# yulong314/multi_camera_calibration

Measured on AMD Instinct MI355X. Metric: corner residual+Jacobian evals/sec + ms/LM-iter; RMS reproj-err vs ref, higher is better.
Workload: dtype f64; 1 GPU; config4: 4 omnidirectional cameras, 1000 synthetic 11x8-board views (BASELINE.json configs[3]), one Gauss-Newton step per 'step'; model=omnidirectional, cameras=4, views=1000, edges=3958, params=6018, parallelism=photo-sharded x1, transport=none, state_dtype=f32, jacobian_dtype=f64

## Files before the change

### multi_camera_calibration_amd/csrc/mcc_group.hpp

```cpp


template <int MODEL, bool BACK, int L, int GW = 28>
__device__ __forceinline__ void group_prologue(const double* ph, const double* ct, const double* sds, int side,
                                               int sub, double* S, double* P, double* Gb) {
    const double* R1 = ph;
    const double* Jr1 = ph + 9;
    const double* T1 = ph + 18;
    const double* R2 = ct;
    const double* Jl2 = ct + 9;
    const double* T2 = ct + 18;
    double* X = S;
    double* W = S + 15;
    for (int e = sub; e < 12; e += L) {
        if (e < 9) {
            const int i = e / 3, j = e % 3;
            X[e] = dot3_nc(R2[i * 3], R1[j], R2[i * 3 + 1], R1[3 + j], R2[i * 3 + 2], R1[6 + j]);
        } else {
            const int i = e - 9;
            const double q = dot3_nc(R2[i * 3], T1[0], R2[i * 3 + 1], T1[1], R2[i * 3 + 2], T1[2]);
            X[12 + i] = q;
            X[9 + i] = add_nc(q, T2[i]);
        }
    }
    wave_sync_lds();
// ... 569 lines not shown
                r[t - ntri] = v;
            }
        }
        if (tid < 2) norms[tid] = a.packed[ntri + 2 * m + tid];
        __syncthreads();
    }
    SSTAMP(srow, 3, 0);
    SolveCtx sc = a.solve;
    sc.stamps = srow;
    solve_global<false>(sc, S, r, norms[0], norms[1], nullptr, ivok ? Iv : nullptr, pre);
    SSTAMP(srow, 7, 0);
    fold_final_reset(la, src, have, useiv);
    SSTAMP_DRAINED(srow, 15, 0);
}
#ifndef MCC_FOLD_EARLY
#define MCC_FOLD_EARLY 1
#endif
template <int NT>
__device__ __forceinline__ void fold_final(const LinArgs& la) {
    __shared__ SolvePre s_pre;
    const SolvePre* pre = MCC_FOLD_EARLY ? &s_pre : nullptr;
    if (MCC_FOLD_EARLY && la.fsa.fuse_solve) {
        SolveCtx sc = la.fsa.solve;
        sc.stamps = la.fsa.stamps ? la.fsa.stamps + kSchurStampStride * (size_t)la.fold_parts : nullptr;
        solve_prefetch(sc, &s_pre);
    }
    if (NT == 512 && la.fold_direct) {
        fold_final_direct(la, pre);
        return;
    }
    constexpr int UM = kSchurOneLevelLoads * 256 / NT;
    const int n = 48 * la.fold_parts + (la.fsa.ssinv != nullptr ? la.fsa.m * la.fsa.m + 1 : 0);
    if (n <= UM / 2 * NT) fold_final_u<UM / 2>(la, pre);
    else fold_final_u<UM>(la, pre);
}

#ifndef MCC_GROUP_PAIR_THREADS
#define MCC_GROUP_PAIR_THREADS 256
#endif
#ifndef MCC_GROUP_OCC
#define MCC_GROUP_OCC 2
#endif
#ifndef MCC_EDGE_PRIO
#define MCC_EDGE_PRIO 2
#endif
template <int L, int AT>
__device__ __forceinline__ void edge_prio_up() {
    if (L == 32 && MCC_EDGE_PRIO == AT && __builtin_amdgcn_readfirstlane(threadIdx.x) >= 256) __builtin_amdgcn_s_setprio(1);
}
template <int L>
__device__ __forceinline__ void edge_prio_down() {
    if (L == 32 && MCC_EDGE_PRIO != 0) __builtin_amdgcn_s_setprio(0);
}
template <int MODEL, bool RATIONAL, int PRISM, bool BACK, int L>
__device__ __forceinline__ bool group_body(const LinArgs& a, const int grp) {
    constexpr int NT = kGroupRound * L, EPW = 64 / L;
    State* st = a.state;
    const int tid = threadIdx.x, lane = tid & 63, wave = tid >> 6;
    const int wv = __builtin_amdgcn_readfirstlane(wave);
    const int* __restrict__ hdr = a.ghdr + (size_t)kGHdrInts * grp;
    const int done = st->done, pending = st->pending;
    const double alpha_prev = st->alpha;
    const int p0 = hdr[kGHdrRange], np = hdr[kGHdrRange + 1];
    const int ge0 = hdr[kGHdrRange + 2], gne = hdr[kGHdrRange + 3];
    const int q0 = hdr[kGHdrRange + 4], nq = hdr[kGHdrRange + 5];
    const int c0 = hdr[kGHdrRange + 6], nc = hdr[kGHdrRange + 7];
    if (done) return false;
    long long* stp = a.stamps ? a.stamps + kStampStride * (size_t)grp : nullptr;
    SSTAMP(stp, 0, 0);
    const int C = a.n_cams, m = a.global_dim;
    extern __shared__ __attribute__((aligned(16))) double smem[];
    const GroupLayout GL = group_layout(gne, C, nq, nc);
#ifdef MCC_DIAG
    long long wt0 = 0, wt1 = 0, wt2 = 0, wt3 = 0;
#endif
    double* rec = smem + GL.rec;
    double* s27 = smem + GL.s27;
    double* sLi = smem + GL.sLi;
    double* sv = smem + GL.sv;
    double* sph = smem + GL.sph;
    double* sxn = smem + GL.sxn;
    double* spart = smem + GL.spart;
    double* sdg = smem + GL.sdg;
    double* ctab = smem + GL.ctab;
    double* ktab = smem + GL.ktab;
    double* sds = smem + GL.sds;
    double* sP = smem + GL.sP;
    double* sGb = smem + GL.sGb;
    int* ibase = reinterpret_cast<int*>(smem + GL.ndoubles);
    int4* sInfo = reinterpret_cast<int4*>(ibase + GL.iInfo);
    int* sgb = ibase + GL.iGb;
    int* seq = ibase + GL.iEq;
    int* sph0 = ibase + GL.iPh;
    int4* spq = reinterpret_cast<int4*>(ibase + GL.iPq);
    unsigned* scn = reinterpret_cast<unsigned*>(ibase + GL.iCn);
    float(*sC)[kGChunk][EPW] = reinterpret_cast<float(*)[kGChunk][EPW]>(smem + GL.sU + wave * (5 * kGChunk * EPW / 2));
    GroupChain* sCH = reinterpret_cast<GroupChain*>(smem + GL.sU + wave * (5 * kGChunk * EPW / 2));
    static_assert(EPW * sizeof(GroupChain) <= 5 * kGChunk * EPW * sizeof(float), "k_group chain union");

    const int g = lane % EPW, sub = lane / EPW;
    constexpr int PER = kGChunk / L;
    auto stage_load = [&](float (&v)[PER][5], int sb, int eoff, int cc0, int cn) {
#pragma unroll
        for (int u = 0; u < PER; ++u) {
            const int i = sb + L * u;
            const unsigned c = (unsigned)(eoff + cc0 + (i < cn ? i : 0));
            v[u][0] = a.obj_x[c];
            v[u][1] = a.obj_y[c];
            v[u][2] = a.obj_z[c];
            v[u][3] = a.img_u[c];
            v[u][4] = a.img_v[c];
        }
    };
    auto stage_store = [&](const float (&v)[PER][5], int sb, int cn) {
#pragma unroll
        for (int u = 0; u < PER; ++u) {
            const int i = sb + L * u;
            if (i < cn) {
#pragma unroll
                for (int f = 0; f < 5; ++f) sC[f][i][g] = v[u][f];
            }
        }
    };
    auto stage = [&](int eoff, int cc0, int cn) {
        float v[PER][5];
        int sb = sub;
        asm volatile("" : "+v"(sb));
        stage_load(v, sb, eoff, cc0, cn);
        stage_store(v, sb, cn);
    };

    constexpr int CAM0 = NT / 2, DST = CAM0 + 63;
    double om2[3] = {0.0, 0.0, 0.0}, T2[3] = {0.0, 0.0, 0.0};
    const int le0 = wave * EPW + g;
    const int4 info0 = *reinterpret_cast<const int4*>(hdr + kGHdrInfo + 4 * le0);
    int4 rInfo = make_int4(0, 0, 0, 0);
    int rGb = 0, rEq = 0, rPh = 0;
    if (wv == 0) {
        const int t = lane < kGroupRound ? lane : 0;
        rInfo = *reinterpret_cast<const int4*>(hdr + kGHdrInfo + 4 * t);
        rGb = hdr[kGHdrGb + t];
        rEq = hdr[kGHdrEq + t];
        rPh = hdr[kGHdrPhoto + (lane <= kPhotoGroup ? lane : 0)];
    }
    int4 rPq = make_int4(0, 0, 0, 0);
    unsigned rCn = 0;
    double rDg = 0.0, rKt = 0.0;
    if (wv * 64 < nq) rPq = a.gpairs[q0 + (tid < nq ? tid : 0)];
    if (wv * 64 < nc) rCn = a.gcon[c0 + (tid < nc ? tid : 0)];
    if (wv * 64 < m) rDg = a.dg[tid < m ? tid : 0];
    if (wv * 64 < kGIntr * C) rKt = a.kintr[tid < kGIntr * C ? tid : 0];
    float rCam[6] = {0.f, 0.f, 0.f, 0.f, 0.f, 0.f};
    double rDs[6] = {0.0, 0.0, 0.0, 0.0, 0.0, 0.0};
    if (wv == CAM0 / 64) {
        const int c = lane < C ? lane : 0;
        const float* src = MODEL == MCC_MODEL_DOUBLESIDE ? a.cam_rt + 6 * c : a.x + 6 * (c > 0 ? c - 1 : 0);
        if (BACK && MODEL == MCC_MODEL_DOUBLESIDE) src = tid == DST ? a.x : src;
#pragma unroll
        for (int k = 0; k < 6; ++k) rCam[k] = src[k];
        if (BACK && MODEL != MCC_MODEL_DOUBLESIDE) {
#pragma unroll
            for (int k = 0; k < 6; ++k) rDs[k] = a.ds_rt[k];
        }
    }
    float xo = 0.f;
    double zk = 0.0;
    const int pq = (tid - 192) / 6, pk = (tid - 192) % 6;
    const bool ptask = tid >= 192 && pq < np;
    double2 pn0 = make_double2(0.0, 0.0);
    if (wv == 3) {
        const size_t pi = ptask ? 6 * (size_t)(p0 + pq) + pk : 0;
        xo = a.x[m + pi];
        if (pending) zk = a.zp[pi];
        else if (a.fold) pn0 = *reinterpret_cast<const double2*>(a.photo_norm + (ptask && pk == 0 ? 2 * (size_t)(p0 + pq) : 0));
    }
    double y0[6] = {0.0, 0.0, 0.0, 0.0, 0.0, 0.0};
    int gb0 = -1;
    if (pending && wv * 64 < 6 * gne) {
        const bool act = tid < 6 * gne;
        const int le = act ? tid / 6 : 0, k = act ? tid % 6 : 0;
        gb0 = a.gblock[ge0 + le];
        const double* Ye = a.Y + 36 * (size_t)(ge0 + le);
#pragma unroll
        for (int i = 0; i < 6; ++i) y0[i] = Ye[6 * i + k];
    }
    float cv0[PER][5];
    int sb0 = sub;
    asm volatile("" : "+v"(sb0));
    const int cn0 = min(info0.w, kGChunk);
    __builtin_amdgcn_sched_barrier(0);
    stage_load(cv0, sb0, info0.z, 0, cn0);
    __builtin_amdgcn_sched_barrier(0);
#pragma unroll
    for (int k = 0; k < 6; ++k) asm volatile("" : "+v"(rCam[k]));
    if (wv == 0) {
        if (lane < kGroupRound && lane < gne) {
            sInfo[lane] = rInfo;
            sgb[lane] = rGb;
            seq[lane] = rEq;
        }
        if (lane <= np) sph0[lane] = rPh;
    }
    if (tid < nq) spq[tid] = rPq;
    if (tid < nc) scn[tid] = rCn;
    if (tid < m) sdg[tid] = rDg;
    if (tid < kGIntr * C) ktab[tid] = rKt;
    if (tid >= CAM0 && tid < CAM0 + C) {
        const bool fixed0 = MODEL != MCC_MODEL_DOUBLESIDE && tid == CAM0;
#pragma unroll
        for (int k = 0; k < 3; ++k) {
            om2[k] = fixed0 ? 0.0 : (double)rCam[k];
            T2[k] = fixed0 ? 0.0 : (double)rCam[3 + k];
        }
    } else if (BACK && tid == DST) {
#pragma unroll
        for (int k = 0; k < 3; ++k) {
            om2[k] = MODEL == MCC_MODEL_DOUBLESIDE ? (double)rCam[k] : rDs[k];
            T2[k] = MODEL == MCC_MODEL_DOUBLESIDE ? (double)rCam[3 + k] : rDs[3 + k];
        }
    }
#pragma unroll 1
    for (int t = kGroupRound + tid; t < gne; t += NT) {
        sInfo[t] = a.edge_info[ge0 + t];
        sgb[t] = a.gblock[ge0 + t];
        seq[t] = a.edge_lphoto[ge0 + t];
    }
#pragma unroll 1
    for (int t = NT + tid; t < nq; t += NT) spq[t] = a.gpairs[q0 + t];
#pragma unroll 1
    for (int t = NT + tid; t < nc; t += NT) scn[t] = a.gcon[c0 + t];
#pragma unroll 1
    for (int t = NT + tid; t < kGIntr * C; t += NT) ktab[t] = a.kintr[t];
    __syncthreads();
    SSTAMP(stp, 1, 0);
    if (pending) {
        for (int t = tid; t < 6 * gne; t += NT) {
            const int le = t / 6, k = t % 6;
            int gbl = gb0;
            double y[6];
            if (t == tid) {
#pragma unroll
                for (int i = 0; i < 6; ++i) y[i] = y0[i];
            } else {
                gbl = sgb[le];
                const double* Ye = a.Y + 36 * (size_t)(ge0 + le);
#pragma unroll
                for (int i = 0; i < 6; ++i) y[i] = Ye[6 * i + k];
            }
            const double* d = sdg + 6 * (gbl < 0 ? 0 : gbl);
            double sk = 0.0;
#pragma unroll
            for (int i = 0; i < 6; ++i) sk += y[i] * d[i];
            spart[6 * le + k] = gbl < 0 ? 0.0 : sk;
        }
    }
    __syncthreads();
    if (tid >= CAM0 && tid < CAM0 + C) {
        const int c = tid - CAM0;
        Rot r2;
        rodrigues_v2m(om2, r2);
        double J[9];
        so3_jac(om2, r2, +1.0, J);
        double* ct = ctab + 24 * c;
#pragma unroll
        for (int k = 0; k < 9; ++k) { ct[k] = r2.R[k]; ct[9 + k] = J[k]; }
#pragma unroll
        for (int k = 0; k < 3; ++k) ct[18 + k] = T2[k];
    } else if (BACK && tid == DST) {
        Rot rd;
        rodrigues_v2m(om2, rd);
        double J[9];
        so3_jac(om2, rd, -1.0, J);
#pragma unroll
        for (int k = 0; k < 9; ++k) { sds[k] = rd.R[k]; sds[9 + k] = J[k]; }
#pragma unroll
        for (int k = 0; k < 3; ++k) sds[18 + k] = T2[k];
    }
    if (ptask) {
        float xn = xo;
        double Gk = 0.0;
        if (pending) {
            double t = zk;
            for (int le = sph0[pq]; le < sph0[pq + 1]; ++le) t -= spart[6 * le + pk];
            const float G = (float)(alpha_prev * t);
            xn = xo + G;
            a.x[m + 6 * (size_t)(p0 + pq) + pk] = xn;
            Gk = (double)G;
        }
        sxn[16 * pq + pk] = (double)xn;
        sxn[16 * pq + 8 + pk] = Gk;
    }
    wave_sync_lds();
    if (ptask && pk == 0) {
        const double* xs = sxn + 16 * pq;
        if (pending) {
            double g2 = 0.0, x2 = 0.0;
#pragma unroll
            for (int q = 0; q < 6; ++q) {
                g2 += xs[8 + q] * xs[8 + q];
                x2 += xs[q] * xs[q];
            }
            a.photo_norm[2 * (size_t)(p0 + pq)] = g2;
            a.photo_norm[2 * (size_t)(p0 + pq) + 1] = x2;
            pn0 = make_double2(g2, x2);
        }
        if (a.fold) {
            sxn[16 * pq + 6] = pn0.x;
            sxn[16 * pq + 7] = pn0.y;
        }
        const double om1[3] = {xs[0], xs[1], xs[2]};
        Rot r1;
        rodrigues_v2m(om1, r1);
        double* ph = sph + 24 * pq;
        so3_jac(om1, r1, -1.0, ph + 9);
#pragma unroll
        for (int k = 0; k < 9; ++k) ph[k] = r1.R[k];
#pragma unroll
        for (int k = 0; k < 3; ++k) ph[18 + k] = xs[3 + k];
    }
    __syncthreads();
    SSTAMP(stp, 2, 0);
    WSTAMP(wt0);
    stage_store(cv0, sb0, cn0);

    for (int rb = 0; rb < gne; rb += kGroupRound) {
        const int es = wave * EPW + g, le = rb + es;
        const bool ev = le < gne;
        const int4 info = ev ? sInfo[le] : make_int4(0, 0, 0, 0);
        const int cam = info.x;
        double* P = sP + kGRecP * es;
        double* Gbe = sGb + 56 * es;
        edge_prio_up<L, 1>();
        if (rb > 0 && ev) stage(info.z, 0, min(info.w, kGChunk));
        if (ev) {
            group_prologue<MODEL, BACK, L>(sph + 24 * seq[le], ctab + 24 * cam, sds, info.y, sub, rec + kGRec * le, P, Gbe);
            const double* kt = ktab + kGIntr * cam;
            for (int k = sub; k < (PRISM == 2 ? 27 : 18); k += L) P[12 + k] = kt[k];
        }
        wave_sync_lds();
        if (rb == 0) SSTAMP(stp, 3, 0);
        if (rb == 0) WSTAMP(wt1);
        edge_prio_up<L, 2>();
        double acc[32];
#pragma unroll
        for (int q = 0; q < 32; ++q) acc[q] = 0.0;
        const int nn = info.w;
        for (int cc0 = 0;; cc0 += kGChunk) {
            if (cc0 >= nn) break;
            const int cn = min(nn - cc0, kGChunk);
            if (cc0 > 0) {
                wave_sync_lds();
                stage(info.z, cc0, cn);
                wave_sync_lds();
            }
#pragma unroll 1
            for (int i = sub; i < cn; i += L) {
                int po = 0;
                asm volatile("" : "+v"(po));
                const double* Pq = P + po;
                double R[9], T[3], kd[12];
#pragma unroll
                for (int q = 0; q < 9; ++q) R[q] = Pq[q];
#pragma unroll
                for (int q = 0; q < 3; ++q) T[q] = Pq[9 + q];
#pragma unroll
                for (int q = 0; q < 12; ++q) kd[q] = Pq[18 + q];
                const double fx = Pq[12], fy = Pq[13], cx = Pq[14], cy = Pq[15], sk = Pq[16], xi = Pq[17];
                const double X = sC[0][i][g], Y = sC[1][i][g], Z = sC[2][i][g];
                const float ou = sC[3][i][g], ov = sC[4][i][g];
                double Yr[3], D[6];
                float u, v;
                if (MODEL == MCC_MODEL_OMNI)
                    omni_corner(R, T, kd, fx, fy, cx, cy, sk, xi, X, Y, Z, Yr, u, v, D);
                else
                    pinhole_corner<RATIONAL, PRISM>(R, T, kd, fx, fy, cx, cy, X, Y, Z, Yr, u, v, D, Pq + 30);
                const float euf = ou - u, evf = ov - v;
                if (a.resid) {
                    const size_t c = (size_t)info.z + cc0 + i;
                    a.resid[2 * c] = euf;
                    a.resid[2 * c + 1] = evf;
                }
                const double eu = euf, ev2 = evf;
                double ju[6], jv[6];
                ju[0] = Yr[1] * D[2] - Yr[2] * D[1];
                ju[1] = Yr[2] * D[0] - Yr[0] * D[2];
                ju[2] = Yr[0] * D[1] - Yr[1] * D[0];
                ju[3] = D[0]; ju[4] = D[1]; ju[5] = D[2];
                jv[0] = Yr[1] * D[5] - Yr[2] * D[4];
                jv[1] = Yr[2] * D[3] - Yr[0] * D[5];
                jv[2] = Yr[0] * D[4] - Yr[1] * D[3];
                jv[3] = D[3]; jv[4] = D[4]; jv[5] = D[5];
                int q = 0;
#pragma unroll
                for (int r = 0; r < 6; ++r)
#pragma unroll
                    for (int s2 = r; s2 < 6; ++s2, ++q) acc[q] = fma(jv[r], jv[s2], fma(ju[r], ju[s2], acc[q]));
#pragma unroll
                for (int r = 0; r < 6; ++r) acc[21 + r] = fma(jv[r], ev2, fma(ju[r], eu, acc[21 + r]));
            }
        }
        if (rb == 0) SSTAMP(stp, 4, 0);
        if (rb == 0) WSTAMP(wt2);
        edge_prio_up<L, 3>();
        int tq = lane;
        asm volatile("" : "+v"(tq));
        strided_reduce_scatter<L>(acc, tq);
        const int gq = tq % EPW, sq = tq / EPW;
        const int base = strided_rs_base<L>(tq);
        wave_sync_lds();
        {
            GroupChain& CW = sCH[gq];
#pragma unroll
            for (int q = 0; q < 32 / L; ++q) {
                const int idx = base + q;
                if (idx < 21) {
                    int r, s2;
                    tri6(idx, r, s2);
                    CW.A[r * 6 + s2] = acc[q];
                    CW.A[s2 * 6 + r] = acc[q];
                } else if (idx < 27) {
                    CW.B[idx - 21] = acc[q];
                }
            }
        }
        wave_sync_lds();
        {
            const int eq = rb + wave * EPW + gq;
            group_chain(sCH[gq], sGb + 56 * (wave * EPW + gq), sq, eq < gne, rec + kGRec * (eq < gne ? eq : 0));
        }
        wave_sync_lds();
        edge_prio_down<L>();
        if (rb == 0) SSTAMP(stp, 5, 0);
        if (rb == 0) WSTAMP(wt3);
// ... 26 lines not shown
        const int q = tid, photo = p0 + q;
        double A[21], gs[6], Lm[6][6], Li[6][6];
        const double2* S2 = reinterpret_cast<const double2*>(s27 + 28 * q);
#pragma unroll
        for (int k = 0; k < 14; ++k) {
            const double2 w = S2[k];
            if (2 * k < 21) A[2 * k] = w.x; else gs[2 * k - 21] = w.x;
            if (2 * k + 1 < 21) A[2 * k + 1] = w.y; else if (2 * k + 1 < 27) gs[2 * k + 1 - 21] = w.y;
        }
        bool bad = false;
        double idg[6];
#pragma unroll
        for (int j = 0; j < 6; ++j) {
            double d = A[6 * j - j * (j - 1) / 2];
#pragma unroll
            for (int k = 0; k < j; ++k) d -= Lm[j][k] * Lm[j][k];
            bad |= !(d > 0.0);
            const double sd = sqrt(d > 0.0 ? d : 1.0);
            const double is = 1.0 / sd;
            Lm[j][j] = sd;
            idg[j] = is;
#pragma unroll
            for (int i = j + 1; i < 6; ++i) {
                double t = A[6 * j - j * (j - 1) / 2 + (i - j)];
#pragma unroll
                for (int k = 0; k < j; ++k) t -= Lm[i][k] * Lm[j][k];
                Lm[i][j] = t * is;
            }
        }
#pragma unroll
        for (int j = 0; j < 6; ++j) {
#pragma unroll
            for (int i = 0; i < 6; ++i) {
                if (i < j) { Li[i][j] = 0.0; continue; }
                double t = i == j ? 1.0 : 0.0;
#pragma unroll
                for (int k = j; k < i; ++k) t -= Lm[i][k] * Li[k][j];
                Li[i][j] = t * idg[i];
            }
        }
        double vv[6];
#pragma unroll
        for (int i = 0; i < 6; ++i) {
            double t = 0.0;
#pragma unroll
            for (int k = 0; k <= i; ++k) t += Li[i][k] * gs[k];
            vv[i] = t;
        }
#pragma unroll
        for (int j = 0; j < 6; ++j) {
            double t = 0.0;
#pragma unroll
            for (int i = j; i < 6; ++i) t += Li[i][j] * vv[i];
            a.zp[6 * (size_t)photo + j] = t;
            a.gp_tot[6 * (size_t)photo + j] = gs[j];
            sv[6 * q + j] = vv[j];
        }
        double2* L2 = reinterpret_cast<double2*>(sLi + 36 * q);
#pragma unroll
        for (int k = 0; k < 18; ++k) L2[k] = make_double2(Li[(2 * k) / 6][(2 * k) % 6], Li[(2 * k + 1) / 6][(2 * k + 1) % 6]);
        if (bad || photo == a.fault_photo) atomicOr(&st->error, kErrPhotoNotPD);
        if (a.fold) {
            double* fw = a.fnorm + 4 * (size_t)photo;
            st_sc1_x2(fw, sxn[16 * q + 6], sxn[16 * q + 7]);
            st_sc1(fw + 2, bad || photo == a.fault_photo ? 1.0 : 0.0);
        }
    }
    __syncthreads();
    SSTAMP(stp, 8, 0);
    for (int t = tid; t < 6 * gne; t += NT) {
        const int le = t / 6, i = t % 6;
        double h[6], li[36], u[6], y[6];
        double2* H2 = reinterpret_cast<double2*>(sE + ES * le + 22 + 6 * i);
        const double2* I2 = reinterpret_cast<const double2*>(sLi + 36 * seq[le]);
#pragma unroll
        for (int q = 0; q < 3; ++q) { const double2 w = H2[q]; h[2 * q] = w.x; h[2 * q + 1] = w.y; }
#pragma unroll
        for (int q = 0; q < 18; ++q) { const double2 w = I2[q]; li[2 * q] = w.x; li[2 * q + 1] = w.y; }
        const bool gl = sgb[le] >= 0;
#pragma unroll
        for (int j = 0; j < 6; ++j) {
            double w = 0.0;
#pragma unroll
            for (int k = 0; k <= j; ++k) w += h[k] * li[6 * j + k];
            u[j] = gl ? w : 0.0;
        }
#pragma unroll
        for (int j = 0; j < 6; ++j) {
            double w = 0.0;
#pragma unroll
            for (int k = j; k < 6; ++k) w += u[k] * li[6 * k + j];
            y[j] = w;
        }
        double2* G2 = reinterpret_cast<double2*>(a.Y + 36 * (size_t)(ge0 + le) + 6 * i);
#pragma unroll
        for (int q = 0; q < 3; ++q) {
            H2[q] = make_double2(u[2 * q], u[2 * q + 1]);
            G2[q] = make_double2(y[2 * q], y[2 * q + 1]);
        }
    }
    __syncthreads();
    SSTAMP(stp, 9, 0);
    int H = 1;
    while (H < 32 && 6 * nq * 2 * H <= (NT < MCC_GROUP_PAIR_THREADS ? NT : MCC_GROUP_PAIR_THREADS)) H *= 2;
    for (int t = tid; t < 6 * nq * H; t += NT) {
        const int h = t % H, k = t / H / 6, i0 = (t / H) % 6;
        const int4 pqv = spq[k];
        const bool diag = (pqv.z & 2) != 0;
        double acc[6], racc = 0.0, jacc = 0.0;
#pragma unroll
        for (int j = 0; j < 6; ++j) acc[j] = 0.0;
#pragma unroll 1
        for (int c = pqv.x + h; c < pqv.x + pqv.y; c += H) {
            const unsigned w = scn[c];
            const int ea = w & 255, eb = (w >> 8) & 255, q = w >> 17;
            const bool self = (w >> 16) & 1;
            const double2* Y2 = reinterpret_cast<const double2*>(sE + ES * ea + 22 + 6 * i0);
            const double2* B2 = reinterpret_cast<const double2*>(sE + ES * eb + 22);
            double y[6];
#pragma unroll
            for (int qq = 0; qq < 3; ++qq) { const double2 v = Y2[qq]; y[2 * qq] = v.x; y[2 * qq + 1] = v.y; }
            const double* Hgg = sE + ES * ea;
#pragma unroll
            for (int j = 0; j < 6; ++j) {
                double hb[6];
#pragma unroll
                for (int qq = 0; qq < 3; ++qq) { const double2 v = B2[3 * j + qq]; hb[2 * qq] = v.x; hb[2 * qq + 1] = v.y; }
                double d = 0.0;
#pragma unroll
                for (int kk = 0; kk < 6; ++kk) d += y[kk] * hb[kk];
                double hv = 0.0;
                if (self) {
                    const int rr = i0 < j ? i0 : j, cc = i0 < j ? j : i0;
                    hv = Hgg[rr * 6 - rr * (rr - 1) / 2 + (cc - rr)];
                }
                acc[j] += self ? hv - d : -d;
            }
            if (diag && self) {
                double d = 0.0;
#pragma unroll
                for (int kk = 0; kk < 6; ++kk) d += y[kk] * sv[6 * q + kk];
                const double gg = sE[ES * ea + 58 + i0];
                racc += gg - d;
                jacc += gg;
            }
        }
        for (int o = 1; o < H; o <<= 1) {
#pragma unroll
            for (int j = 0; j < 6; ++j) acc[j] += __shfl_xor(acc[j], o);
            racc += __shfl_xor(racc, o);
            jacc += __shfl_xor(jacc, o);
        }
        if (h == 0) {
            double* out = a.pairprod + (size_t)pqv.w;
#ifdef MCC_SLOT_PLAIN
#pragma unroll
            for (int j = 0; j < 6; ++j) out[i0 * 6 + j] = acc[j];
            if (diag) {
                out[36 + i0] = racc;
                out[42 + i0] = jacc;
            }
#else
#pragma unroll
            for (int j = 0; j < 6; j += 2) st_sc1_x2(out + i0 * 6 + j, acc[j], acc[j + 1]);
            if (diag) {
                st_sc1(out + 36 + i0, racc);
                st_sc1(out + 42 + i0, jacc);
            }
#endif
        }
    }
#ifdef MCC_DIAG
    asm volatile("s_waitcnt vmcnt(0)" ::: "memory");
    __syncthreads();
    SSTAMP(stp, 10, 0);
#endif
    return true;
}

template <int MODEL, bool RATIONAL, int PRISM, bool BACK, int L, bool FIRST = false>
__global__ __launch_bounds__(kGroupRound * L, MCC_GROUP_OCC * 16 / L) void k_group(LinArgs a) {
    constexpr int NT = kGroupRound * L;
    static_assert(L == 16 || L == 32, "k_group: 16 or 32 lanes per edge");
    State* st = a.state;
    const int tid = threadIdx.x;
    int grp = blockIdx.x;
    if (FIRST) {
        const int nlead = (int)gridDim.x - a.n_pgroups;
        grp = grp < nlead ? a.n_pgroups + grp : grp - nlead;
    }
    if (a.ssinv && grp == a.n_pgroups) {
        extern __shared__ __attribute__((aligned(16))) double smem_spare[];
        small_inverse(a, smem_spare, false);
        return;
    }
    int task;
    if (a.fold && grp > a.n_pgroups - (a.ssinv ? 0 : 1)) {
        if (st->done) return;
        task = grp - a.n_pgroups - (a.ssinv ? 1 : 0);
    } else {
        if (!group_body<MODEL, RATIONAL, PRISM, BACK, L>(a, grp) || PRISM == 2 || !a.fold_dyn) return;
        __shared__ int s_task;
        __syncthreads();
        if (tid == 0) {
            const int t = __hip_atomic_fetch_add(a.fold_ticket, 1, __ATOMIC_RELAXED, __HIP_MEMORY_SCOPE_AGENT);
            if (t == a.n_pgroups - 1) __hip_atomic_store(a.fold_ticket, 0, __ATOMIC_RELAXED, __HIP_MEMORY_SCOPE_AGENT);
            s_task = t;
        }
        __syncthreads();
        task = s_task;
    }
    if (task < a.fsa.n_items) fold_item(a, task);
    else if (task < a.fold_parts) fold_chunk(a, task - a.fsa.n_items);
    else if (task == a.fold_parts) fold_final<NT>(a);
}

#ifndef MCC_PREP4_WAVES
#define MCC_PREP4_WAVES 2
#endif
template <int MODEL, bool BACK>
__global__ __launch_bounds__(64, MCC_PREP4_WAVES) void k_prep4(LinArgs a) {
    const State* st = a.state;
    const int tid = threadIdx.x, grp = blockIdx.x;
    const int done = st->done, pending = st->pending;
    const double alpha_prev = st->alpha;
    const int p0 = a.prep_ptr[grp], np = a.prep_ptr[grp + 1] - p0;
    const int ge0 = a.prep_edge[grp], gne = a.prep_edge[grp + 1] - ge0;
    if (done) return;
    long long* stp = a.stamps ? a.stamps + kStampStride * (size_t)grp + 8 : nullptr;
    SSTAMP(stp, 0, 0);
    const int C = a.n_cams, m = a.global_dim;
    extern __shared__ __attribute__((aligned(16))) double smem[];
    const PrepLayout PL = prep_layout(C, BACK);
    double* tab = smem + PL.tab;
    double* S = smem + PL.S;
    double* spart = S;
    double* sdg = smem + PL.sdg;
    double* sxn = smem + PL.sxn;
    double* scam = smem + PL.scam;
    int* ib = reinterpret_cast<int*>(smem + PL.ndoubles);
    int4* sInfo = reinterpret_cast<int4*>(ib + PL.iInfo);
    int* sgb = ib + PL.iGb;
    int* sph0 = ib + PL.iPh;
    constexpr int SW = BACK ? 84 : 42;
    for (int t = tid; t < m; t += 64) sdg[t] = a.dg[t];
    for (int t = tid; t < 6 * C; t += 64) {
        const int c = t / 6, k = t % 6;
        scam[t] = MODEL == MCC_MODEL_DOUBLESIDE ? (double)a.cam_rt[t]
                                                : (c == 0 ? 0.0 : (double)a.x[6 * (c - 1) + k]);
    }
    if (BACK && tid < 6) scam[6 * C + tid] = MODEL == MCC_MODEL_DOUBLESIDE ? (double)a.x[tid] : a.ds_rt[tid];
    if (tid <= np) sph0[tid] = a.photo_ptr[p0 + tid] - ge0;
    for (int t = tid; t < gne; t += 64) {
        sInfo[t] = a.edge_info[ge0 + t];
        sgb[t] = a.gblock[ge0 + t];
    }
    const int pq = tid / 6, pk = tid % 6;
    const bool ptask = pq < np;
    float xo = 0.f;
    double zk = 0.0;
    double2 pn0 = make_double2(0.0, 0.0);
    if (ptask) {
        xo = a.x[m + 6 * (size_t)(p0 + pq) + pk];
        if (pending) zk = a.zp[6 * (size_t)(p0 + pq) + pk];
        else if (a.fold && pk == 0) pn0 = *reinterpret_cast<const double2*>(a.photo_norm + 2 * (size_t)(p0 + pq));
    }
    double y0[6];
// ... 100 lines not shown
```

### multi_camera_calibration_amd/csrc/mcc_internal.h

```cpp
#pragma once
#include <hip/hip_runtime.h>

#include "../../include/mcc.h"
#include "mcc_layout.hpp"

namespace mcc {

constexpr int kStampStride = 32;
constexpr int kSchurStampStride = 16;

struct State {
    int iter;
    int done;
    int crit_type;
    int max_count;
    double eps;
    double change;
    double alpha;
    double cam_normG2, cam_normX2;
    int error;
    int pending;
    unsigned int epoch;
    long long xchg_ticks;
    unsigned int spare_ack;
};
constexpr int kErrPhotoNotPD = 1;
constexpr int kErrCameraNotPD = 2;
constexpr int kErrPeerTimeout = 4;
constexpr int kErrWarmTimeout = 8;

struct PeerCtx {
    unsigned long long* inbox;
    unsigned long long* const* peers;
    int nranks;
    int rank, Lc;
    long long timeout;
};

struct SolveCtx {
    State* state;
    const double* alpha; int n_alpha;
    float* x;
    double* dg;
    double* delta;
    int m, do_update;
    long long* stamps;
    long long* sstats;
};

struct SchurArgs {
    State* state;
    const int4* items;
    const double* pairprod;
    double* item_out;
// ... 29 lines not shown
    const float* K; const float* D; const float* xi;
    const double* tilt;
    const float* cam_rt;
    const double* ds_rt;
    int nd, global_dim, n_cams, has_back;
    double* Y;
    const int* pgrp_ptr;
    const int* pgrp_edge;
    const unsigned char* edge_lphoto;
    const int* gpair_ptr;
    const int4* gpairs;
    const int* gcon_ptr;
    const unsigned* gcon;
    double* pairprod;
    int n_pgroups, max_gpairs, max_gcon, max_gedges;
    double* zp;
    double* gp_tot;
    float* resid;
    const int* gblock;
    const double* dg;
    double* photo_norm;
    long long* stamps;
    int fused, group_size, n_groups, rank, fuse_solve;
    double* contrib;
    double* gsum;
    int* cnt;
    double* packed;
    double* W;
    SolveCtx solve;
    PeerCtx peer;
    int n_edges, n_photos;
    double* erec;
    double* echain;
    double* eh;
    const int* prep_ptr;
    const int* prep_edge;
    int n_prep, prep_lanes;
    int fault_photo;
    int fold_first;
    double* ssinv;
    int* ssinv_ok;
    long long spare_wait, spare_delay;
    int fold, fold_parts;
    int fold_direct;
    int fold_dyn;
    int* fold_ticket;
    SchurArgs fsa;
    double* fnorm;
    double* fiv;
    const int* ghdr;
    const double* kintr;
};

struct WarmCtx {
    double* sinv;
    int* sinv_ok_sys;
    double* prev2;
    int prev_stride;
    int copy_prev;
    unsigned* sync;
    long long* stats;
    int poison;
    long long wait_ticks;
    long long idle_ticks;
    long long delay_ticks;
    int refine;
    double* xsol;
    int poll;
    long long* hst;
    int inv_la;
};
constexpr int kWarmMaxIters = 4;

struct SolveArgs {
    SolveCtx ctx;
    double* packed;
    PeerCtx peer;
    int pushed;
    WarmCtx warm;
};

struct BacksubArgs {
    const State* state;
    const int* photo_ptr;
    const int* gblock;
    const double* Y; const double* zp; const double* dg;
    const double* W;
    float* x;
    double* delta;
    double* photo_norm;
    int n_photos, m, do_update;
};

struct ErrArgs {
    const int4* edge_info;
    const int* edge_photo;
    const float* obj_x; const float* obj_y; const float* obj_z;
    const float* img_u; const float* img_v;
    const float* x;
    const float* K; const float* D; const float* xi;
    const double* tilt;
    const float* cam_pose;
    float* edge_sum;
    float* corner_err;
    int nd, m;
};
// ... 22 lines not shown
```

### multi_camera_calibration_amd/csrc/mcc_kernels.hip

```cpp
#include <array>
#include <map>
#include <mutex>
#include <hip/hip_runtime.h>

#include <algorithm>

#include "mcc_device.hpp"
#include "mcc_internal.h"

#ifdef MCC_PART
#define MCC_IN(n) (MCC_PART == (n))
#else
#define MCC_IN(n) 1
#endif
hipError_t mcc_attrs_linearize(size_t shmem);
hipError_t mcc_attrs_group16(size_t shmem);
hipError_t mcc_attrs_group32(size_t shmem);
hipError_t mcc_attrs_photo(size_t shmem);
hipError_t mcc_attrs_solve(size_t shmem);

namespace mcc {

#ifdef MCC_DIAG_RT
#define MCC_DIAG_CLOCK() __builtin_amdgcn_s_memrealtime()
// ... 4012 lines not shown
        if (p4) hipLaunchKernelGGL((k_prep4<MCC_MODEL_OMNI, false>), g4, dim3(64), p4shm, s, a);
        else hipLaunchKernelGGL((k_prep<MCC_MODEL_OMNI, false>), gp, dim3(64), 0, s, a);
        launch_edge<MCC_MODEL_OMNI, false, false>(a, s);
    } else if (model == MCC_MODEL_DOUBLESIDE) {
        if (p4) hipLaunchKernelGGL((k_prep4<MCC_MODEL_DOUBLESIDE, true>), g4, dim3(64), p4shm, s, a);
        else hipLaunchKernelGGL((k_prep<MCC_MODEL_DOUBLESIDE, true>), gp, dim3(64), 0, s, a);
        if (prism == 2) launch_edge<MCC_MODEL_DOUBLESIDE, true, 2>(a, s);
        else if (rational && prism) launch_edge<MCC_MODEL_DOUBLESIDE, true, true>(a, s);
        else if (rational) launch_edge<MCC_MODEL_DOUBLESIDE, true, false>(a, s);
        else if (prism) launch_edge<MCC_MODEL_DOUBLESIDE, false, true>(a, s);
        else launch_edge<MCC_MODEL_DOUBLESIDE, false, false>(a, s);
    } else {
        if (p4 && a.has_back) hipLaunchKernelGGL((k_prep4<MCC_MODEL_PINHOLE, true>), g4, dim3(64), p4shm, s, a);
        else if (p4) hipLaunchKernelGGL((k_prep4<MCC_MODEL_PINHOLE, false>), g4, dim3(64), p4shm, s, a);
        else if (a.has_back) hipLaunchKernelGGL((k_prep<MCC_MODEL_PINHOLE, true>), gp, dim3(64), 0, s, a);
        else hipLaunchKernelGGL((k_prep<MCC_MODEL_PINHOLE, false>), gp, dim3(64), 0, s, a);
        if (prism == 2) launch_edge<MCC_MODEL_PINHOLE, true, 2>(a, s);
        else if (rational && prism) launch_edge<MCC_MODEL_PINHOLE, true, true>(a, s);
        else if (rational) launch_edge<MCC_MODEL_PINHOLE, true, false>(a, s);
        else if (prism) launch_edge<MCC_MODEL_PINHOLE, false, true>(a, s);
        else launch_edge<MCC_MODEL_PINHOLE, false, false>(a, s);
    }
    hipLaunchKernelGGL(k_photo, dim3(a.n_pgroups), dim3(256), photo_shmem, s, a);
    return hipGetLastError();
}
hipError_t mcc_attrs_photo(size_t shmem) {
    return hipFuncSetAttribute((const void*)&k_photo, hipFuncAttributeMaxDynamicSharedMemorySize, (int)shmem);
}
#endif

#if MCC_IN(0)

size_t mcc_lin_shmem(int max_edges_per_photo, int n_cams, int m, int max_cpp) {
    const size_t lin = (size_t)max_edges_per_photo * sizeof(EdgeLds) + sizeof(PhotoLds) +
                       (kCamStride + kIntrStride) * sizeof(double) * (size_t)n_cams +
                       ((5 * sizeof(float) * (size_t)max_cpp + 15) & ~(size_t)15);
    return std::max(lin, (size_t)((m <= 30 ? 2 : 1) * m * m + m) * sizeof(double));
}

size_t mcc_solve_shmem(int m) {
    const size_t M = 16 * (size_t)((m + 15) / 16);
    const size_t blocked = M + M * (M + 1) + 2 * 16 * kBlkLd;
    const size_t warm = M <= kWarmN ? kWarmN + warm_shmem_doubles(m) : 0;
    const size_t helper = M <= kWarmN ? helper_shmem_doubles(m, true) : 0;
    return std::max((size_t)(m * m + m), m > 30 ? std::max(std::max(blocked, warm), helper) : 0) * sizeof(double);
}

#endif

#if MCC_IN(2) || MCC_IN(3)
template <int MODEL, bool RATIONAL, int PRISM, bool BACK, int L>
static hipError_t launch_group_t(const LinArgs& a, size_t shmem, hipStream_t s) {
    const dim3 grid(a.n_pgroups + (a.ssinv ? 1 : 0) + (a.fold && !a.fold_dyn ? a.fold_parts + 1 : 0));
    if (a.fold_first) {
        if (MODEL != MCC_MODEL_OMNI) return hipErrorInvalidValue;
        hipLaunchKernelGGL((k_group<MCC_MODEL_OMNI, false, false, false, L, true>), grid, dim3(kGroupRound * L), shmem, s, a);
        return hipGetLastError();
    }
    hipLaunchKernelGGL((k_group<MODEL, RATIONAL, PRISM, BACK, L>), grid, dim3(kGroupRound * L), shmem, s, a);
    return hipGetLastError();
}
template <int L>
static hipError_t launch_group_l(const LinArgs& a, int model, bool rational, int prism, size_t shmem, hipStream_t s) {
    if (model == MCC_MODEL_OMNI) return launch_group_t<MCC_MODEL_OMNI, false, false, false, L>(a, shmem, s);
    if (model == MCC_MODEL_DOUBLESIDE) {
        if (prism == 2) return launch_group_t<MCC_MODEL_DOUBLESIDE, true, 2, true, L>(a, shmem, s);
        if (rational && prism) return launch_group_t<MCC_MODEL_DOUBLESIDE, true, true, true, L>(a, shmem, s);
        if (rational) return launch_group_t<MCC_MODEL_DOUBLESIDE, true, false, true, L>(a, shmem, s);
        if (prism) return launch_group_t<MCC_MODEL_DOUBLESIDE, false, true, true, L>(a, shmem, s);
        return launch_group_t<MCC_MODEL_DOUBLESIDE, false, false, true, L>(a, shmem, s);
    }
    if (a.has_back) {
        if (prism == 2) return launch_group_t<MCC_MODEL_PINHOLE, true, 2, true, L>(a, shmem, s);
        if (rational && prism) return launch_group_t<MCC_MODEL_PINHOLE, true, true, true, L>(a, shmem, s);
        if (rational) return launch_group_t<MCC_MODEL_PINHOLE, true, false, true, L>(a, shmem, s);
        if (prism) return launch_group_t<MCC_MODEL_PINHOLE, false, true, true, L>(a, shmem, s);
        return launch_group_t<MCC_MODEL_PINHOLE, false, false, true, L>(a, shmem, s);
    }
    if (prism == 2) return launch_group_t<MCC_MODEL_PINHOLE, true, 2, false, L>(a, shmem, s);
    if (rational && prism) return launch_group_t<MCC_MODEL_PINHOLE, true, true, false, L>(a, shmem, s);
    if (rational) return launch_group_t<MCC_MODEL_PINHOLE, true, false, false, L>(a, shmem, s);
    if (prism) return launch_group_t<MCC_MODEL_PINHOLE, false, true, false, L>(a, shmem, s);
    return launch_group_t<MCC_MODEL_PINHOLE, false, false, false, L>(a, shmem, s);
}
template <int L>
static hipError_t set_group_attrs(size_t group_shmem) {
    hipError_t err = hipSuccess;
#define SETG(M, R, P, B) hipFuncSetAttribute((const void*)&k_group<M, R, P, B, L>, hipFuncAttributeMaxDynamicSharedMemorySize, (int)group_shmem)
    for (hipError_t e : {SETG(1, false, false, false), SETG(2, true, true, true), SETG(2, true, false, true),
                         SETG(2, false, true, true), SETG(2, false, false, true), SETG(0, true, true, true),
                         SETG(0, true, false, true), SETG(0, false, true, true), SETG(0, false, false, true),
                         SETG(0, true, true, false), SETG(0, true, false, false), SETG(0, false, true, false),
                         SETG(0, false, false, false), SETG(2, true, 2, true), SETG(0, true, 2, true),
                         SETG(0, true, 2, false),
                         hipFuncSetAttribute((const void*)&k_group<1, false, false, false, L, true>,
                                             hipFuncAttributeMaxDynamicSharedMemorySize, (int)group_shmem)})
        if (e != hipSuccess) err = e;
#undef SETG
    return err;
}
#endif
#if MCC_IN(3)
hipError_t mcc_launch_group32(const LinArgs& a, int model, bool rational, int prism, size_t shmem, hipStream_t s) {
    return launch_group_l<32>(a, model, rational, prism, shmem, s);
}
hipError_t mcc_attrs_group32(size_t shmem) { return set_group_attrs<32>(shmem); }
#endif
#if MCC_IN(2)
hipError_t mcc_launch_group32(const LinArgs& a, int model, bool rational, int prism, size_t shmem, hipStream_t s);
hipError_t mcc_launch_group(const LinArgs& a, int model, bool rational, int prism, int lanes, size_t shmem,
                            hipStream_t s) {
    if (a.n_photos <= 0 || a.n_edges <= 0) return hipSuccess;
// ... 119 lines not shown
```

Baseline: 14.31 billion corner evals/s.

## Restructure k_group kernel arguments into lead/hot blocks pinned in scalar registers

Splits k_group's single LinArgs argument into a 64-byte leading block of scalars, the full LinArgs, and a compact GroupHot struct of frequently used pointers. The kernel reads these straight from the kernarg segment at compile-time offsets and uses asm constraints to keep header values and pointers in SGPRs, with readfirstlane on the uniform state loads. The aim is to cut scalar load latency and vector register pressure in the group prologue. It also adds fragile offset bookkeeping guarded by static_asserts, and it enlarges the argument segment.

```diff
diff --git a/multi_camera_calibration_amd/csrc/mcc_group.hpp b/multi_camera_calibration_amd/csrc/mcc_group.hpp
--- a/multi_camera_calibration_amd/csrc/mcc_group.hpp
+++ b/multi_camera_calibration_amd/csrc/mcc_group.hpp
@@ -645,23 +645,60 @@
 __device__ __forceinline__ void edge_prio_down() {
     if (L == 32 && MCC_EDGE_PRIO != 0) __builtin_amdgcn_s_setprio(0);
 }
+template <class T>
+__device__ __forceinline__ T* pin_global(T* p) {
+    __attribute__((address_space(1))) T* g = (__attribute__((address_space(1))) T*)p;
+    asm volatile("" : "+s"(g));
+    return (T*)g;
+}
+__device__ __forceinline__ int first_lane(int v) { return __builtin_amdgcn_readfirstlane(v); }
+__device__ __forceinline__ double first_lane(double v) {
+    return __hiloint2double(first_lane(__double2hiint(v)), first_lane(__double2loint(v)));
+}
+template <class T>
+__device__ __forceinline__ const T& kernarg_at(const int off) {
+    typedef const __attribute__((address_space(4))) char* kbytes;
+    const __attribute__((address_space(4))) T* p =
+        (const __attribute__((address_space(4))) T*)((kbytes)__builtin_amdgcn_kernarg_segment_ptr() + off);
+    asm volatile("" : "+s"(p));
+    return *(const T*)p;
+}
 template <int MODEL, bool RATIONAL, int PRISM, bool BACK, int L>
-__device__ __forceinline__ bool group_body(const LinArgs& a, const int grp) {
+__device__ __forceinline__ bool group_body(State* st, const int* __restrict__ ghdr, const bool fold, const int grp,
+                                           const long long t_entry) {
     constexpr int NT = kGroupRound * L, EPW = 64 / L;
-    State* st = a.state;
     const int tid = threadIdx.x, lane = tid & 63, wave = tid >> 6;
     const int wv = __builtin_amdgcn_readfirstlane(wave);
-    const int* __restrict__ hdr = a.ghdr + (size_t)kGHdrInts * grp;
-    const int done = st->done, pending = st->pending;
-    const double alpha_prev = st->alpha;
-    const int p0 = hdr[kGHdrRange], np = hdr[kGHdrRange + 1];
-    const int ge0 = hdr[kGHdrRange + 2], gne = hdr[kGHdrRange + 3];
-    const int q0 = hdr[kGHdrRange + 4], nq = hdr[kGHdrRange + 5];
-    const int c0 = hdr[kGHdrRange + 6], nc = hdr[kGHdrRange + 7];
+    const int* __restrict__ hdr = ghdr + (size_t)kGHdrInts * grp;
+    int done = first_lane(st->done), pending = first_lane(st->pending);
+    double alpha_prev = first_lane(st->alpha);
+    int p0 = first_lane(hdr[kGHdrRange]), np = first_lane(hdr[kGHdrRange + 1]);
+    int ge0 = first_lane(hdr[kGHdrRange + 2]), gne = first_lane(hdr[kGHdrRange + 3]);
+    int q0 = first_lane(hdr[kGHdrRange + 4]), nq = first_lane(hdr[kGHdrRange + 5]);
+    int c0 = first_lane(hdr[kGHdrRange + 6]), nc = first_lane(hdr[kGHdrRange + 7]);
+    GroupHot hp = kernarg_at<GroupHot>(kGArgHot);
+    asm volatile("" ::"s"(done), "s"(pending), "s"(alpha_prev), "s"(p0), "s"(np), "s"(ge0), "s"(gne), "s"(q0), "s"(nq),
+                 "s"(c0), "s"(nc), "s"(hp.gpairs), "s"(hp.gcon), "s"(hp.dg), "s"(hp.kintr), "s"(hp.x), "s"(hp.cam_rt),
+                 "s"(hp.ds_rt), "s"(hp.zp), "s"(hp.photo_norm), "s"(hp.gblock), "s"(hp.Y), "s"(hp.obj_x), "s"(hp.obj_y),
+                 "s"(hp.obj_z), "s"(hp.img_u), "s"(hp.img_v), "s"(hp.stamps), "s"(hp.global_dim), "s"(hp.n_cams));
+    asm volatile("" ::"s"(hp.edge_info), "s"(hp.edge_lphoto), "s"(hp.gp_tot), "s"(hp.resid));
+    asm volatile("" : "+s"(done), "+s"(pending), "+s"(alpha_prev), "+s"(p0), "+s"(np), "+s"(ge0), "+s"(gne), "+s"(q0),
+                 "+s"(nq), "+s"(c0), "+s"(nc), "+s"(hp.global_dim), "+s"(hp.n_cams));
+    hp.gpairs = pin_global(hp.gpairs); hp.gcon = pin_global(hp.gcon); hp.dg = pin_global(hp.dg);
+    hp.kintr = pin_global(hp.kintr); hp.x = pin_global(hp.x); hp.cam_rt = pin_global(hp.cam_rt);
+    hp.ds_rt = pin_global(hp.ds_rt); hp.zp = pin_global(hp.zp); hp.photo_norm = pin_global(hp.photo_norm);
+    hp.gblock = pin_global(hp.gblock); hp.Y = pin_global(hp.Y); hp.obj_x = pin_global(hp.obj_x);
+    hp.obj_y = pin_global(hp.obj_y); hp.obj_z = pin_global(hp.obj_z); hp.img_u = pin_global(hp.img_u);
+    hp.img_v = pin_global(hp.img_v); hp.stamps = pin_global(hp.stamps);
+    hp.edge_info = pin_global(hp.edge_info); hp.edge_lphoto = pin_global(hp.edge_lphoto);
+    hp.gp_tot = pin_global(hp.gp_tot); hp.resid = pin_global(hp.resid);
     if (done) return false;
-    long long* stp = a.stamps ? a.stamps + kStampStride * (size_t)grp : nullptr;
+    long long* stp = hp.stamps ? hp.stamps + kStampStride * (size_t)grp : nullptr;
     SSTAMP(stp, 0, 0);
-    const int C = a.n_cams, m = a.global_dim;
+#ifdef MCC_DIAG
+    if (stp && (tid == 0 || tid == NT - 64)) stp[tid == 0 ? 12 : 13] = t_entry;
+#endif
+    const int C = hp.n_cams, m = hp.global_dim;
     extern __shared__ __attribute__((aligned(16))) double smem[];
     const GroupLayout GL = group_layout(gne, C, nq, nc);
 #ifdef MCC_DIAG
@@ -698,11 +735,11 @@
         for (int u = 0; u < PER; ++u) {
             const int i = sb + L * u;
             const unsigned c = (unsigned)(eoff + cc0 + (i < cn ? i : 0));
-            v[u][0] = a.obj_x[c];
-            v[u][1] = a.obj_y[c];
-            v[u][2] = a.obj_z[c];
-            v[u][3] = a.img_u[c];
-            v[u][4] = a.img_v[c];
+            v[u][0] = hp.obj_x[c];
+            v[u][1] = hp.obj_y[c];
+            v[u][2] = hp.obj_z[c];
+            v[u][3] = hp.img_u[c];
+            v[u][4] = hp.img_v[c];
         }
     };
     auto stage_store = [&](const float (&v)[PER][5], int sb, int cn) {
@@ -739,21 +776,21 @@
     int4 rPq = make_int4(0, 0, 0, 0);
     unsigned rCn = 0;
     double rDg = 0.0, rKt = 0.0;
-    if (wv * 64 < nq) rPq = a.gpairs[q0 + (tid < nq ? tid : 0)];
-    if (wv * 64 < nc) rCn = a.gcon[c0 + (tid < nc ? tid : 0)];
-    if (wv * 64 < m) rDg = a.dg[tid < m ? tid : 0];
-    if (wv * 64 < kGIntr * C) rKt = a.kintr[tid < kGIntr * C ? tid : 0];
+    if (wv * 64 < nq) rPq = hp.gpairs[q0 + (tid < nq ? tid : 0)];
+    if (wv * 64 < nc) rCn = hp.gcon[c0 + (tid < nc ? tid : 0)];
+    if (wv * 64 < m) rDg = hp.dg[tid < m ? tid : 0];
+    if (wv * 64 < kGIntr * C) rKt = hp.kintr[tid < kGIntr * C ? tid : 0];
     float rCam[6] = {0.f, 0.f, 0.f, 0.f, 0.f, 0.f};
     double rDs[6] = {0.0, 0.0, 0.0, 0.0, 0.0, 0.0};
     if (wv == CAM0 / 64) {
         const int c = lane < C ? lane : 0;
-        const float* src = MODEL == MCC_MODEL_DOUBLESIDE ? a.cam_rt + 6 * c : a.x + 6 * (c > 0 ? c - 1 : 0);
-        if (BACK && MODEL == MCC_MODEL_DOUBLESIDE) src = tid == DST ? a.x : src;
+        const float* src = MODEL == MCC_MODEL_DOUBLESIDE ? hp.cam_rt + 6 * c : hp.x + 6 * (c > 0 ? c - 1 : 0);
+        if (BACK && MODEL == MCC_MODEL_DOUBLESIDE) src = tid == DST ? hp.x : src;
 #pragma unroll
         for (int k = 0; k < 6; ++k) rCam[k] = src[k];
         if (BACK && MODEL != MCC_MODEL_DOUBLESIDE) {
 #pragma unroll
-            for (int k = 0; k < 6; ++k) rDs[k] = a.ds_rt[k];
+            for (int k = 0; k < 6; ++k) rDs[k] = hp.ds_rt[k];
         }
     }
     float xo = 0.f;
@@ -763,17 +800,17 @@
     double2 pn0 = make_double2(0.0, 0.0);
     if (wv == 3) {
         const size_t pi = ptask ? 6 * (size_t)(p0 + pq) + pk : 0;
-        xo = a.x[m + pi];
-        if (pending) zk = a.zp[pi];
-        else if (a.fold) pn0 = *reinterpret_cast<const double2*>(a.photo_norm + (ptask && pk == 0 ? 2 * (size_t)(p0 + pq) : 0));
+        xo = hp.x[m + pi];
+        if (pending) zk = hp.zp[pi];
+        else if (fold) pn0 = *reinterpret_cast<const double2*>(hp.photo_norm + (ptask && pk == 0 ? 2 * (size_t)(p0 + pq) : 0));
     }
     double y0[6] = {0.0, 0.0, 0.0, 0.0, 0.0, 0.0};
     int gb0 = -1;
     if (pending && wv * 64 < 6 * gne) {
         const bool act = tid < 6 * gne;
         const int le = act ? tid / 6 : 0, k = act ? tid % 6 : 0;
-        gb0 = a.gblock[ge0 + le];
-        const double* Ye = a.Y + 36 * (size_t)(ge0 + le);
+        gb0 = hp.gblock[ge0 + le];
+        const double* Ye = hp.Y + 36 * (size_t)(ge0 + le);
 #pragma unroll
         for (int i = 0; i < 6; ++i) y0[i] = Ye[6 * i + k];
     }
@@ -814,18 +851,19 @@
     }
 #pragma unroll 1
     for (int t = kGroupRound + tid; t < gne; t += NT) {
-        sInfo[t] = a.edge_info[ge0 + t];
-        sgb[t] = a.gblock[ge0 + t];
-        seq[t] = a.edge_lphoto[ge0 + t];
+        sInfo[t] = hp.edge_info[ge0 + t];
+        sgb[t] = hp.gblock[ge0 + t];
+        seq[t] = hp.edge_lphoto[ge0 + t];
     }
 #pragma unroll 1
-    for (int t = NT + tid; t < nq; t += NT) spq[t] = a.gpairs[q0 + t];
+    for (int t = NT + tid; t < nq; t += NT) spq[t] = hp.gpairs[q0 + t];
 #pragma unroll 1
-    for (int t = NT + tid; t < nc; t += NT) scn[t] = a.gcon[c0 + t];
+    for (int t = NT + tid; t < nc; t += NT) scn[t] = hp.gcon[c0 + t];
 #pragma unroll 1
-    for (int t = NT + tid; t < kGIntr * C; t += NT) ktab[t] = a.kintr[t];
+    for (int t = NT + tid; t < kGIntr * C; t += NT) ktab[t] = hp.kintr[t];
     __syncthreads();
     SSTAMP(stp, 1, 0);
+    const LinArgs& a = kernarg_at<LinArgs>(kGArgLin);
     if (pending) {
         for (int t = tid; t < 6 * gne; t += NT) {
             const int le = t / 6, k = t % 6;
@@ -836,7 +874,7 @@
                 for (int i = 0; i < 6; ++i) y[i] = y0[i];
             } else {
                 gbl = sgb[le];
-                const double* Ye = a.Y + 36 * (size_t)(ge0 + le);
+                const double* Ye = hp.Y + 36 * (size_t)(ge0 + le);
 #pragma unroll
                 for (int i = 0; i < 6; ++i) y[i] = Ye[6 * i + k];
             }
@@ -877,7 +915,7 @@
             for (int le = sph0[pq]; le < sph0[pq + 1]; ++le) t -= spart[6 * le + pk];
             const float G = (float)(alpha_prev * t);
             xn = xo + G;
-            a.x[m + 6 * (size_t)(p0 + pq) + pk] = xn;
+            hp.x[m + 6 * (size_t)(p0 + pq) + pk] = xn;
             Gk = (double)G;
         }
         sxn[16 * pq + pk] = (double)xn;
@@ -893,11 +931,11 @@
                 g2 += xs[8 + q] * xs[8 + q];
                 x2 += xs[q] * xs[q];
             }
-            a.photo_norm[2 * (size_t)(p0 + pq)] = g2;
-            a.photo_norm[2 * (size_t)(p0 + pq) + 1] = x2;
+            hp.photo_norm[2 * (size_t)(p0 + pq)] = g2;
+            hp.photo_norm[2 * (size_t)(p0 + pq) + 1] = x2;
             pn0 = make_double2(g2, x2);
         }
-        if (a.fold) {
+        if (fold) {
             sxn[16 * pq + 6] = pn0.x;
             sxn[16 * pq + 7] = pn0.y;
         }
@@ -968,10 +1006,10 @@
                 else
                     pinhole_corner<RATIONAL, PRISM>(R, T, kd, fx, fy, cx, cy, X, Y, Z, Yr, u, v, D, Pq + 30);
                 const float euf = ou - u, evf = ov - v;
-                if (a.resid) {
+                if (hp.resid) {
                     const size_t c = (size_t)info.z + cc0 + i;
-                    a.resid[2 * c] = euf;
-                    a.resid[2 * c + 1] = evf;
+                    hp.resid[2 * c] = euf;
+                    hp.resid[2 * c + 1] = evf;
                 }
                 const double eu = euf, ev2 = evf;
                 double ju[6], jv[6];
@@ -1104,15 +1142,15 @@
             double t = 0.0;
 #pragma unroll
             for (int i = j; i < 6; ++i) t += Li[i][j] * vv[i];
-            a.zp[6 * (size_t)photo + j] = t;
-            a.gp_tot[6 * (size_t)photo + j] = gs[j];
+            hp.zp[6 * (size_t)photo + j] = t;
+            hp.gp_tot[6 * (size_t)photo + j] = gs[j];
             sv[6 * q + j] = vv[j];
         }
         double2* L2 = reinterpret_cast<double2*>(sLi + 36 * q);
 #pragma unroll
         for (int k = 0; k < 18; ++k) L2[k] = make_double2(Li[(2 * k) / 6][(2 * k) % 6], Li[(2 * k + 1) / 6][(2 * k + 1) % 6]);
         if (bad || photo == a.fault_photo) atomicOr(&st->error, kErrPhotoNotPD);
-        if (a.fold) {
+        if (fold) {
             double* fw = a.fnorm + 4 * (size_t)photo;
             st_sc1_x2(fw, sxn[16 * q + 6], sxn[16 * q + 7]);
             st_sc1(fw + 2, bad || photo == a.fault_photo ? 1.0 : 0.0);
@@ -1144,7 +1182,7 @@
             for (int k = j; k < 6; ++k) w += u[k] * li[6 * k + j];
             y[j] = w;
         }
-        double2* G2 = reinterpret_cast<double2*>(a.Y + 36 * (size_t)(ge0 + le) + 6 * i);
+        double2* G2 = reinterpret_cast<double2*>(hp.Y + 36 * (size_t)(ge0 + le) + 6 * i);
 #pragma unroll
         for (int q = 0; q < 3; ++q) {
             H2[q] = make_double2(u[2 * q], u[2 * q + 1]);
@@ -1231,40 +1269,50 @@
 }
 
 template <int MODEL, bool RATIONAL, int PRISM, bool BACK, int L, bool FIRST = false>
-__global__ __launch_bounds__(kGroupRound * L, MCC_GROUP_OCC * 16 / L) void k_group(LinArgs a) {
+__global__ __launch_bounds__(kGroupRound * L, MCC_GROUP_OCC * 16 / L) void k_group(
+    State* st, const int* ghdr, const int n_pgroups, const unsigned flags, const int n_items, const int fold_parts,
+    long long, long long, long long, long long, LinArgs, GroupHot) {
     constexpr int NT = kGroupRound * L;
     static_assert(L == 16 || L == 32, "k_group: 16 or 32 lanes per edge");
-    State* st = a.state;
+    static_assert(GSame<decltype(&k_group<MODEL, RATIONAL, PRISM, BACK, L, FIRST>), GroupKernelFn>::v,
+                  "k_group's parameters are GroupKernelFn's: kernarg_at's offsets are computed from that list");
+    long long t_entry = 0;
+    WSTAMP(t_entry);
     const int tid = threadIdx.x;
+    const bool spare = (flags & kGLeadSsinv) != 0, fold = (flags & kGLeadFold) != 0;
     int grp = blockIdx.x;
     if (FIRST) {
-        const int nlead = (int)gridDim.x - a.n_pgroups;
-        grp = grp < nlead ? a.n_pgroups + grp : grp - nlead;
-    }
-    if (a.ssinv && grp == a.n_pgroups) {
+        const int nlead = (int)gridDim.x - n_pgroups;
+        grp = grp < nlead ? n_pgroups + grp : grp - nlead;
+    }
+    if (spare && grp == n_pgroups) {
         extern __shared__ __attribute__((aligned(16))) double smem_spare[];
-        small_inverse(a, smem_spare, false);
+        small_inverse(kernarg_at<LinArgs>(kGArgLin), smem_spare, false);
         return;
     }
     int task;
-    if (a.fold && grp > a.n_pgroups - (a.ssinv ? 0 : 1)) {
+    if (fold && grp > n_pgroups - (spare ? 0 : 1)) {
         if (st->done) return;
-        task = grp - a.n_pgroups - (a.ssinv ? 1 : 0);
+        task = grp - n_pgroups - (spare ? 1 : 0);
     } else {
-        if (!group_body<MODEL, RATIONAL, PRISM, BACK, L>(a, grp) || PRISM == 2 || !a.fold_dyn) return;
+        if (!group_body<MODEL, RATIONAL, PRISM, BACK, L>(st, ghdr, fold, grp, t_entry) || PRISM == 2 ||
+            !(flags & kGLeadFoldDyn))
+            return;
         __shared__ int s_task;
         __syncthreads();
         if (tid == 0) {
-            const int t = __hip_atomic_fetch_add(a.fold_ticket, 1, __ATOMIC_RELAXED, __HIP_MEMORY_SCOPE_AGENT);
-            if (t == a.n_pgroups - 1) __hip_atomic_store(a.fold_ticket, 0, __ATOMIC_RELAXED, __HIP_MEMORY_SCOPE_AGENT);
+            int* ticket = kernarg_at<LinArgs>(kGArgLin).fold_ticket;
+            const int t = __hip_atomic_fetch_add(ticket, 1, __ATOMIC_RELAXED, __HIP_MEMORY_SCOPE_AGENT);
+            if (t == n_pgroups - 1) __hip_atomic_store(ticket, 0, __ATOMIC_RELAXED, __HIP_MEMORY_SCOPE_AGENT);
             s_task = t;
         }
         __syncthreads();
         task = s_task;
     }
-    if (task < a.fsa.n_items) fold_item(a, task);
-    else if (task < a.fold_parts) fold_chunk(a, task - a.fsa.n_items);
-    else if (task == a.fold_parts) fold_final<NT>(a);
+    const LinArgs& a = kernarg_at<LinArgs>(kGArgLin);
+    if (task < n_items) fold_item(a, task);
+    else if (task < fold_parts) fold_chunk(a, task - n_items);
+    else if (task == fold_parts) fold_final<NT>(a);
 }
 
 #ifndef MCC_PREP4_WAVES
diff --git a/multi_camera_calibration_amd/csrc/mcc_internal.h b/multi_camera_calibration_amd/csrc/mcc_internal.h
--- a/multi_camera_calibration_amd/csrc/mcc_internal.h
+++ b/multi_camera_calibration_amd/csrc/mcc_internal.h
@@ -1,5 +1,7 @@
 #pragma once
 #include <hip/hip_runtime.h>
+
+#include <cstddef>
 
 #include "../../include/mcc.h"
 #include "mcc_layout.hpp"
@@ -135,6 +137,82 @@
     const double* kintr;
 };
 
+constexpr unsigned kGLeadSsinv = 1u, kGLeadFold = 2u, kGLeadFoldDyn = 4u, kGLeadFoldDirect = 8u;
+constexpr int kGLeadPreload = 6;
+struct GroupLead {
+    State* state;
+    const int* ghdr;
+    int n_pgroups;
+    unsigned flags;
+    int n_items;
+    int fold_parts;
+    long long pad[4];
+};
+static_assert(sizeof(GroupLead) == 64 && sizeof(GroupLead) % alignof(LinArgs) == 0,
+              "k_group: LinArgs follows the leading block at byte 64 of the argument segment");
+inline GroupLead group_lead(const LinArgs& a) {
+    return {a.state, a.ghdr, a.n_pgroups,
+            (a.ssinv ? kGLeadSsinv : 0u) | (a.fold ? kGLeadFold : 0u) | (a.fold_dyn ? kGLeadFoldDyn : 0u) |
+                (a.fold_direct ? kGLeadFoldDirect : 0u),
+            a.fsa.n_items, a.fold_parts, {0, 0, 0, 0}};
+}
+struct GroupHot {
+    const int4* gpairs;
+    const unsigned* gcon;
+    const double* dg;
+    const double* kintr;
+    float* x;
+    const float* cam_rt;
+    const double* ds_rt;
+    double* zp;
+    double* photo_norm;
+    const int* gblock;
+    double* Y;
+    const float* obj_x; const float* obj_y; const float* obj_z;
+    const float* img_u; const float* img_v;
+    long long* stamps;
+    const int4* edge_info;
+    const unsigned char* edge_lphoto;
+    double* gp_tot;
+    float* resid;
+    int global_dim, n_cams;
+};
+inline GroupHot group_hot(const LinArgs& a) {
+    return {a.gpairs, a.gcon, a.dg, a.kintr, a.x, a.cam_rt, a.ds_rt, a.zp, a.photo_norm, a.gblock, a.Y,
+            a.obj_x, a.obj_y, a.obj_z, a.img_u, a.img_v, a.stamps, a.edge_info, a.edge_lphoto, a.gp_tot, a.resid,
+            a.global_dim, a.n_cams};
+}
+using GroupKernelFn = void (*)(State*, const int*, int, unsigned, int, int, long long, long long, long long, long long,
+                               LinArgs, GroupHot);
+template <class T, class U> struct GSame { static constexpr bool v = false; };
+template <class T> struct GSame<T, T> { static constexpr bool v = true; };
+template <class T, class... P>
+constexpr int kernarg_offset_of(void (*)(P...)) {
+    const size_t sz[] = {sizeof(P)...}, al[] = {alignof(P)...};
+    const bool is[] = {GSame<T, P>::v...};
+    size_t off = 0;
+    for (size_t i = 0; i < sizeof...(P); ++i) {
+        off = (off + al[i] - 1) / al[i] * al[i];
+        if (is[i]) return (int)off;
+        off += sz[i];
+    }
+    return -1;
+}
+constexpr int kGArgLin = kernarg_offset_of<LinArgs>(GroupKernelFn(nullptr));
+constexpr int kGArgHot = kernarg_offset_of<GroupHot>(GroupKernelFn(nullptr));
+struct GroupKernarg {
+    GroupLead lead;
+    LinArgs a;
+    GroupHot hot;
+};
+static_assert(kGArgLin == (int)offsetof(GroupKernarg, a) && kGArgLin == (int)sizeof(GroupLead) && kGArgLin % 64 == 0,
+              "k_group: LinArgs follows the 64-byte leading block");
+static_assert(kGArgHot == (int)offsetof(GroupKernarg, hot) && kGArgHot == kGArgLin + (int)sizeof(LinArgs),
+              "k_group: GroupHot follows LinArgs without padding");
+static_assert(kernarg_offset_of<unsigned>(GroupKernelFn(nullptr)) == (int)offsetof(GroupLead, flags) &&
+                  kernarg_offset_of<long long>(GroupKernelFn(nullptr)) == (int)offsetof(GroupLead, pad),
+              "k_group: the leading parameters lie as GroupLead's members do");
+
 struct WarmCtx {
     double* sinv;
     int* sinv_ok_sys;
diff --git a/multi_camera_calibration_amd/csrc/mcc_kernels.hip b/multi_camera_calibration_amd/csrc/mcc_kernels.hip
--- a/multi_camera_calibration_amd/csrc/mcc_kernels.hip
+++ b/multi_camera_calibration_amd/csrc/mcc_kernels.hip
@@ -4088,12 +4088,17 @@
 template <int MODEL, bool RATIONAL, int PRISM, bool BACK, int L>
 static hipError_t launch_group_t(const LinArgs& a, size_t shmem, hipStream_t s) {
     const dim3 grid(a.n_pgroups + (a.ssinv ? 1 : 0) + (a.fold && !a.fold_dyn ? a.fold_parts + 1 : 0));
+    const GroupLead gl = group_lead(a);
+    const GroupHot gh = group_hot(a);
+#define MCC_GROUP_ARGS gl.state, gl.ghdr, gl.n_pgroups, gl.flags, gl.n_items, gl.fold_parts, 0LL, 0LL, 0LL, 0LL, a, gh
     if (a.fold_first) {
         if (MODEL != MCC_MODEL_OMNI) return hipErrorInvalidValue;
-        hipLaunchKernelGGL((k_group<MCC_MODEL_OMNI, false, false, false, L, true>), grid, dim3(kGroupRound * L), shmem, s, a);
+        hipLaunchKernelGGL((k_group<MCC_MODEL_OMNI, false, false, false, L, true>), grid, dim3(kGroupRound * L), shmem, s,
+                           MCC_GROUP_ARGS);
         return hipGetLastError();
     }
-    hipLaunchKernelGGL((k_group<MODEL, RATIONAL, PRISM, BACK, L>), grid, dim3(kGroupRound * L), shmem, s, a);
+    hipLaunchKernelGGL((k_group<MODEL, RATIONAL, PRISM, BACK, L>), grid, dim3(kGroupRound * L), shmem, s, MCC_GROUP_ARGS);
+#undef MCC_GROUP_ARGS
     return hipGetLastError();
 }
 template <int L>
```

New measurement: 14.65 billion corner evals/s (median of 6 runs). 2.3% higher.
